# GuoleiSun/VSS-CFFM

Measured on AMD Instinct MI355X. Metric: clips/sec (fwd+bwd) CFFM-B1 480x480 T=4 hot path (CFFA+CFM, decoder_focal depth 2), higher is better.
Workload: dtype f32 in/out, f32 accumulate; MFMA operands: split-bf16 (hi+lo, ~2^-17) in the Linear GEMMs, f16 in QK^T/AV

## Files before the change

vss_cffm_amd/csrc/cffa_kernels.h:

```cpp
#pragma once
#include "cffm_common.h"

__device__ __forceinline__ void transpose_body(const float* __restrict__ src, float* __restrict__ dst,
                                               int rows, int cols, long src_bs, long dst_bs,
                                               const float* __restrict__ addend, int add_mod, int add_skip,
                                               float* __restrict__ copy_dst, int bx, int by, int bz) {
    __shared__ float tile[64][65];
    const int r0 = by * 64, c0 = bx * 64;
    const float* s = src + (long)bz * src_bs;
    float* d = dst + (long)bz * dst_bs;
    const int q = threadIdx.x & 15, p = threadIdx.x >> 4;
    const bool vin = (cols % 4 == 0) && (src_bs % 4 == 0) && (((uintptr_t)src & 15) == 0);
    const bool vout = (rows % 4 == 0) && (dst_bs % 4 == 0) && (((uintptr_t)dst & 15) == 0) && (((uintptr_t)addend & 15) == 0);
    const float* ad = (addend && (bz % add_mod) != add_skip) ? addend + (long)bz * dst_bs : nullptr;
    float* cp = (copy_dst && (bz % add_mod) != add_skip) ? copy_dst + (long)bz * src_bs : nullptr;
#pragma unroll
    for (int k = 0; k < 4; ++k) {
        const int r = r0 + p + 16 * k, c = c0 + 4 * q;
        f32x4 v = (f32x4){0.f, 0.f, 0.f, 0.f};
        if (r < rows) {
            if (vin && c + 3 < cols) {
                v = *(const f32x4*)(s + (long)r * cols + c);
                if (cp) *(f32x4*)(cp + (long)r * cols + c) = v;
            } else
                for (int e = 0; e < 4; ++e)
                    if (c + e < cols) { v[e] = s[(long)r * cols + c + e]; if (cp) cp[(long)r * cols + c + e] = v[e]; }
        }
#pragma unroll
        for (int e = 0; e < 4; ++e) tile[4 * q + e][p + 16 * k] = v[e];
    }
    __syncthreads();
#pragma unroll
    for (int k = 0; k < 4; ++k) {
        const int cl = p + 16 * k, c = c0 + cl, r = r0 + 4 * q;
        f32x4 v;
#pragma unroll
        for (int e = 0; e < 4; ++e) v[e] = tile[cl][4 * q + e];
        if (c < cols) {
            if (vout && r + 3 < rows) *(f32x4*)(d + (long)c * rows + r) = ad ? v + *(const f32x4*)(ad + (long)c * rows + r) : v;
            else
                for (int e = 0; e < 4; ++e)
                    if (r + e < rows) d[(long)c * rows + r + e] = v[e] + (ad ? ad[(long)c * rows + r + e] : 0.f);
        }
    }
}
__global__ void __launch_bounds__(256) k_transpose(const float* __restrict__ src, float* __restrict__ dst,
                                                    int rows, int cols, long src_bs, long dst_bs,
                                                    const float* __restrict__ addend, int add_mod, int add_skip,
                                                    float* __restrict__ copy_dst = nullptr) {
    transpose_body(src, dst, rows, cols, src_bs, dst_bs, addend, add_mod, add_skip, copy_dst, blockIdx.x, blockIdx.y, blockIdx.z);
}

__device__ __forceinline__ float bil_tap(int r, int p) {
    if (p == r) return (11.f - 2.f * r) * (1.f / 12.f);
    if (p == r + 1) return (1.f + 2.f * r) * (1.f / 12.f);
    return 0.f;
}

__device__ __forceinline__ void cell_geom(int g, int& grp, int& u, int& v, int& wsg) {
    if (g == 0) { grp = 0; u = v = 0; wsg = 7; }
    else if (g == 1) { grp = 1; u = v = 0; wsg = 7; }
    else if (g < 6) { grp = 2; u = (g - 2) >> 1; v = (g - 2) & 1; wsg = 3; }
    else { grp = 3; u = (g - 6) / 3; v = (g - 6) % 3; wsg = 2; }
}

struct PoolW { const float* w[4]; };
struct PoolWG { float* w[4]; float* b[4]; };

__device__ __forceinline__ float pool_matrix_entry(const PoolW& pw, int g, int i) {
    const int py = i / 7, px = i % 7;
    int grp, u, v, wsg;
    cell_geom(g, grp, u, v, wsg);
    if (grp < 2) return pw.w[grp][i];
    float m = 0.f;
    for (int a = 0; a < wsg; ++a)
        for (int b = 0; b < wsg; ++b)
            m += pw.w[grp][a * wsg + b] * bil_tap(wsg * u + a, py) * bil_tap(wsg * v + b, px);
    return m;
}
__device__ __forceinline__ void pool_matrix_body(const PoolW& pw, float* __restrict__ M) {
    for (int e = threadIdx.x; e < CFFM_NCELL * CFFM_WA; e += 256) M[e] = pool_matrix_entry(pw, e / CFFM_WA, e % CFFM_WA);
}

__global__ void __launch_bounds__(256) k_pool_matrix(PoolW pw, float* __restrict__ M) { pool_matrix_body(pw, M); }

__device__ __forceinline__ void pool_matrix_bwd_body(const float* __restrict__ dM, const PoolWG& gw, int t) {
    const int i = threadIdx.x;
    int grp, k;
    if (t < 49) { grp = 0; k = t; }
    else if (t < 98) { grp = 1; k = t - 49; }
    else if (t < 107) { grp = 2; k = t - 98; }
    else { grp = 3; k = t - 107; }
    float acc = 0.f;
    if (grp < 2) {
        if (i == k) acc = dM[grp * CFFM_WA + k];
    } else if (i < CFFM_WA) {
        const int wsg = grp == 2 ? 3 : 2, ncell = grp == 2 ? 2 : 3, g0 = grp == 2 ? 2 : 6;
        const int a = k / wsg, b = k % wsg;
        for (int u = 0; u < ncell; ++u)
            for (int v = 0; v < ncell; ++v)
                acc += dM[(g0 + u * ncell + v) * CFFM_WA + i] * bil_tap(wsg * u + a, i / 7) * bil_tap(wsg * v + b, i % 7);
    }
    acc = wave_sum(acc);
    if (i == 0) gw.w[grp][k] = acc;
    if (t == 0 && i < 3 && gw.b[0]) {
        gw.w[0][49 + i] = 0.f; gw.w[1][49 + i] = 0.f; gw.w[2][9 + i] = 0.f;
#pragma unroll
        for (int q = 0; q < 4; ++q) gw.b[q][1 + i] = 0.f;
    }
}
#define PMB_MAXD 4
struct PoolWGN { const float* dM[PMB_MAXD]; PoolWG gw[PMB_MAXD]; };
__global__ void __launch_bounds__(64) k_pool_matrix_bwd_n(PoolWGN a) { pool_matrix_bwd_body(a.dM[blockIdx.y], a.gw[blockIdx.y], blockIdx.x); }

struct Geo {
    int B, H0, W0, Hp, Wp, gy, gx, nW, HW, RC;
};
__device__ __forceinline__ int cell_row(const Geo& G, int wy, int wx, int g) {
    const int w = wy * G.gx + wx;
    if (g == 0) return 49 * G.nW + w;
    if (g == 1) return 50 * G.nW + w;
    if (g < 6) { int u = (g - 2) >> 1, v = (g - 2) & 1; return 51 * G.nW + (2 * wy + u) * (2 * G.gx) + 2 * wx + v; }
    int u = (g - 6) / 3, v = (g - 6) % 3;
    return 55 * G.nW + (3 * wy + u) * (3 * G.gx) + 3 * wx + v;
}
__device__ __forceinline__ void frame_cells(int frame, int& g0, int& ncell) {
    if (frame == 3) { g0 = 0; ncell = 1; }
    else if (frame == 0) { g0 = 1; ncell = 1; }
    else if (frame == 1) { g0 = 2; ncell = 4; }
    else { g0 = 6; ncell = 9; }
}

struct PoolB { const float* b[4]; };
struct PoolBG { float* b[4]; };
__device__ __forceinline__ int frame_group(int frame) { return frame == 3 ? 0 : frame + 1; }

#ifndef LNPF_BATCH
#define LNPF_BATCH 4
#endif
#ifndef LNP_WAVES
#define LNP_WAVES 8
#endif
#define LNP_THREADS (64 * LNP_WAVES)
#define LNP_PIX ((CFFM_WA + LNP_WAVES - 1) / LNP_WAVES)
template <bool INFER>
__global__ void __launch_bounds__(LNP_THREADS, 6) k_ln_pool_fwd(Geo G, const float* __restrict__ x_ref, long ref_bs,
                                                      const float* __restrict__ x_tgt, long tgt_bs,
                                                      const float* __restrict__ gamma, const float* __restrict__ beta,
                                                      const float* __restrict__ M , PoolW pw, PoolB pb,
                                                      float* __restrict__ zall, float* __restrict__ mean_out,
                                                      float* __restrict__ rstd_out, int split ) {
    __shared__ float sM[9 * CFFM_WA];
    __shared__ float red[4][9][CFFM_C];
    const int w = blockIdx.x, frame = blockIdx.y, b = blockIdx.z;
    const int wy = w / G.gx, wx = w % G.gx;
    const int lane = threadIdx.x & 63, wave = threadIdx.x >> 6;
    int g0, ncell;
    frame_cells(frame, g0, ncell);
    for (int e = threadIdx.x; e < ncell * CFFM_WA; e += LNP_THREADS)
        sM[e] = (INFER || M) ? M[g0 * CFFM_WA + e] : pool_matrix_entry(pw, g0 + e / CFFM_WA, e % CFFM_WA);
    __syncthreads();
    const float* xf = (frame == 3) ? x_tgt + (long)b * tgt_bs : x_ref + (long)b * ref_bs + (long)frame * G.HW * CFFM_C;
    const f32x4 gm = *(const f32x4*)(gamma + 4 * lane), bt = *(const f32x4*)(beta + 4 * lane);
    f32x4 acc[9];
#pragma unroll
    for (int c = 0; c < 9; ++c) acc[c] = (f32x4){0.f, 0.f, 0.f, 0.f};
#pragma unroll
    for (int k0 = 0; k0 < LNP_PIX; k0 += LNPF_BATCH) {
        f32x4 xr[LNPF_BATCH];
#pragma unroll
        for (int kk = 0; kk < LNPF_BATCH; ++kk) {
            const int i = wave + LNP_WAVES * (k0 + kk);
            const int y = 7 * wy + i / 7, x = 7 * wx + i % 7;
            xr[kk] = (f32x4){0.f, 0.f, 0.f, 0.f};
            if (k0 + kk < LNP_PIX && i < CFFM_WA && y < G.H0 && x < G.W0) xr[kk] = *(const f32x4*)(xf + ((long)y * G.W0 + x) * CFFM_C + 4 * lane);
        }
#pragma unroll
        for (int kk = 0; kk < LNPF_BATCH; ++kk) {
            const int i = wave + LNP_WAVES * (k0 + kk);
            if (k0 + kk >= LNP_PIX || i >= CFFM_WA) break;
            const int y = 7 * wy + i / 7, x = 7 * wx + i % 7;
            const bool valid = (y < G.H0) && (x < G.W0);
            f32x4 z = (f32x4){0.f, 0.f, 0.f, 0.f};
            if (valid) {
                const long pix = (long)y * G.W0 + x;
                const f32x4 xv = xr[kk];
                const float mu = wave_sum(xv[0] + xv[1] + xv[2] + xv[3]) * (1.f / CFFM_C);
                const f32x4 d = xv - mu;
                const float var = wave_sum(d[0] * d[0] + d[1] * d[1] + d[2] * d[2] + d[3] * d[3]) * (1.f / CFFM_C);
                const float rs = 1.f / sqrtf(var + CFFM_LN_EPS);
                z = d * rs * gm + bt;
                if (!INFER && lane == 0) {
                    mean_out[((long)b * 4 + frame) * G.HW + pix] = mu;
                    rstd_out[((long)b * 4 + frame) * G.HW + pix] = rs;
                }
            }
            if (frame == 3) *(f32x4*)(zall + ((long)b * G.RC + w * CFFM_WA + i) * CFFM_C + 4 * lane) = split ? split4_pack(z) : z;
            if (valid) {
#pragma unroll
                for (int c = 0; c < 9; ++c)
                    if (c < ncell) acc[c] += sM[c * CFFM_WA + i] * z;
            }
        }
    }
    static_assert(LNP_WAVES == 4 || LNP_WAVES == 8, "LNP_WAVES");
    if (wave < 4) {
#pragma unroll
        for (int c = 0; c < 9; ++c)
            if (c < ncell) *(f32x4*)(&red[wave][c][4 * lane]) = acc[c];
    }
    __syncthreads();
    if (LNP_WAVES == 8) {
        if (wave >= 4) {
#pragma unroll
            for (int c = 0; c < 9; ++c)
                if (c < ncell) *(f32x4*)(&red[wave - 4][c][4 * lane]) += acc[c];
        }
        __syncthreads();
    }
    const float pbias = pb.b[frame_group(frame)][0];
    if (!split) {
        for (int c = 0; c < ncell && threadIdx.x < CFFM_C; ++c) {
            const int ch = threadIdx.x;
            const float s = red[0][c][ch] + red[1][c][ch] + red[2][c][ch] + red[3][c][ch] + pbias;
            zall[((long)b * G.RC + cell_row(G, wy, wx, g0 + c)) * CFFM_C + ch] = s;
        }
    } else {
        for (int e = threadIdx.x; e < ncell * (CFFM_C / 4); e += LNP_THREADS) {
            const int c = e / (CFFM_C / 4), c4 = 4 * (e % (CFFM_C / 4));
            const f32x4 s = *(const f32x4*)(&red[0][c][c4]) + *(const f32x4*)(&red[1][c][c4]) + *(const f32x4*)(&red[2][c][c4]) +
                            *(const f32x4*)(&red[3][c][c4]) + pbias;
            *(f32x4*)(zall + ((long)b * G.RC + cell_row(G, wy, wx, g0 + c)) * CFFM_C + c4) = split4_pack(s);
        }
    }
}

#define LNP_RSTRIDE 1216
#define LNP_TAIL_TGT (CFFM_WA + 1)
#define LNP_TAIL_REF (14 * CFFM_WA + 3)
#ifndef LNB_SPLIT
#define LNB_SPLIT 4
#endif
#ifndef LNB_WAVES
#define LNB_WAVES 4
#endif
#define LNB_THREADS (64 * LNB_WAVES)
#define LNB_PIX ((CFFM_WA + LNB_SPLIT * LNB_WAVES - 1) / (LNB_SPLIT * LNB_WAVES))

__device__ __forceinline__ float dot4(f32x4 a, f32x4 b) { return a[0] * b[0] + a[1] * b[1] + a[2] * b[2] + a[3] * b[3]; }

__global__ void __launch_bounds__(LNB_THREADS) k_ln_pool_bwd_tgt(Geo G, const float* __restrict__ x_tgt, long tgt_bs,
                                                                 const float* __restrict__ gamma, const float* __restrict__ beta,
                                                                 const float* __restrict__ M, const float* __restrict__ mean_in,
                                                                 const float* __restrict__ rstd_in, const float* __restrict__ dzall,
                                                                 const float* __restrict__ dres, float* __restrict__ dx_tgt, long dtgt_bs,
                                                                 float* __restrict__ rec) {
    __shared__ float red[LNB_WAVES][2][CFFM_C];
    __shared__ float sdM[CFFM_WA];
    __shared__ float sbs;
    const int s = blockIdx.x % LNB_SPLIT, wb = blockIdx.x / LNB_SPLIT;
    const int w = wb % G.nW, b = wb / G.nW;
    const int wy = w / G.gx, wx = w % G.gx;
    const int lane = threadIdx.x & 63, wave = wave_uniform(threadIdx.x >> 6);
    const float* xf = x_tgt + (long)b * tgt_bs;
    float* dxf = dx_tgt + (long)b * dtgt_bs;
    if (threadIdx.x < CFFM_WA) sdM[threadIdx.x] = 0.f;
    f32x4 xr[LNB_PIX], dzr[LNB_PIX], addr[LNB_PIX];
    float mur[LNB_PIX], rsr[LNB_PIX], m0[LNB_PIX];
#pragma unroll
    for (int k = 0; k < LNB_PIX; ++k) {
        const int i = s + LNB_SPLIT * (wave + LNB_WAVES * k);
        const int y = 7 * wy + i / 7, x = 7 * wx + i % 7;
        xr[k] = dzr[k] = addr[k] = (f32x4){0.f, 0.f, 0.f, 0.f};
        mur[k] = rsr[k] = m0[k] = 0.f;
        if (i < CFFM_WA && y < G.H0 && x < G.W0) {
            const long pix = (long)y * G.W0 + x;
            xr[k] = *(const f32x4*)(xf + pix * CFFM_C + 4 * lane);
            mur[k] = mean_in[((long)b * 4 + 3) * G.HW + pix];
            rsr[k] = rstd_in[((long)b * 4 + 3) * G.HW + pix];
            m0[k] = M[i];
            dzr[k] = *(const f32x4*)(dzall + ((long)b * G.RC + w * CFFM_WA + i) * CFFM_C + 4 * lane);
            if (dres) addr[k] = *(const f32x4*)(dres + ((long)b * G.HW + pix) * CFFM_C + 4 * lane);
        }
    }
    const f32x4 dp = *(const f32x4*)(dzall + ((long)b * G.RC + cell_row(G, wy, wx, 0)) * CFFM_C + 4 * lane);
    const f32x4 gm = *(const f32x4*)(gamma + 4 * lane), bt = *(const f32x4*)(beta + 4 * lane);
    if (wave == 0) {
        const float bs = wave_sum(dp[0] + dp[1] + dp[2] + dp[3]);
        if (lane == 0) sbs = (s == 0) ? bs : 0.f;
    }
    f32x4 ag = (f32x4){0.f, 0.f, 0.f, 0.f}, ab = (f32x4){0.f, 0.f, 0.f, 0.f};
    __syncthreads();
#pragma unroll
    for (int k = 0; k < LNB_PIX; ++k) {
        const int i = s + LNB_SPLIT * (wave + LNB_WAVES * k);
        if (i >= CFFM_WA) break;
        const int y = 7 * wy + i / 7, x = 7 * wx + i % 7;
        if (!((y < G.H0) && (x < G.W0))) continue;
        const long pix = (long)y * G.W0 + x;
        const float rs = rsr[k];
        const f32x4 xh = (xr[k] - mur[k]) * rs;
        const f32x4 z = xh * gm + bt;
        const f32x4 dz = dzr[k] + m0[k] * dp;
        const float dm = wave_sum_hi(dot4(dp, z));
        if (lane == 63) sdM[i] = dm;
        ag += dz * xh;
        ab += dz;
        const f32x4 gz = dz * gm;
        const float m1 = wave_sum(gz[0] + gz[1] + gz[2] + gz[3]) * (1.f / CFFM_C);
        const float m2 = wave_sum(dot4(gz, xh)) * (1.f / CFFM_C);
        const f32x4 dx = (gz - m1 - xh * m2) * rs + addr[k];
        *(f32x4*)(dxf + pix * CFFM_C + 4 * lane) = dx;
    }
    *(f32x4*)(&red[wave][0][4 * lane]) = ag;
    *(f32x4*)(&red[wave][1][4 * lane]) = ab;
    __syncthreads();
    float* r = rec + (long)blockIdx.x * LNP_RSTRIDE;
    for (int e = threadIdx.x; e < 2 * CFFM_C; e += LNB_THREADS) {
        const int which = e / CFFM_C, ch = e % CFFM_C;
        float t = red[0][which][ch];
#pragma unroll
        for (int q = 1; q < LNB_WAVES; ++q) t += red[q][which][ch];
        r[e] = t;
    }
    if (threadIdx.x < CFFM_WA) r[2 * CFFM_C + threadIdx.x] = sdM[threadIdx.x];
    if (threadIdx.x == CFFM_WA) r[2 * CFFM_C + CFFM_WA] = sbs;
}

#define RB_MAXD 4
struct CffaRefBlocks {
    int n;
    const float* gamma[RB_MAXD];
    const float* beta[RB_MAXD];
    const float* M[RB_MAXD];
    const float* dzall[RB_MAXD];
    float* rec[RB_MAXD];
};
#define RB_LDS_BLOCK (14 * CFFM_C + 2 * 14 * CFFM_WA)
__host__ __device__ constexpr int cffa_ref_lds(int D) {
    return 4 * ((D * RB_LDS_BLOCK > LNB_WAVES * D * 2 * CFFM_C + 14 * D * CFFM_WA ? D * RB_LDS_BLOCK : LNB_WAVES * D * 2 * CFFM_C + 14 * D * CFFM_WA) + 4 * D + 4);
}

struct RefRows { f32x4 x[LNB_PIX], add[LNB_PIX]; float mu[LNB_PIX], rs[LNB_PIX]; };
template <bool ACC>
__device__ __forceinline__ void ln_pool_ref_load(RefRows& R, const Geo& G, const float* __restrict__ xf, const float* __restrict__ dxf,
                                                 const float* __restrict__ mean_f, const float* __restrict__ rstd_f, int s, int wy, int wx,
                                                 int lane, int wave) {
#pragma unroll
    for (int k = 0; k < LNB_PIX; ++k) {
        const int i = s + LNB_SPLIT * (wave + LNB_WAVES * k);
        const int y = 7 * wy + i / 7, x = 7 * wx + i % 7;
        R.x[k] = R.add[k] = (f32x4){0.f, 0.f, 0.f, 0.f};
        R.mu[k] = R.rs[k] = 0.f;
        if (i < CFFM_WA && y < G.H0 && x < G.W0) {
            const long pix = (long)y * G.W0 + x;
            R.x[k] = *(const f32x4*)(xf + pix * CFFM_C + 4 * lane);
            R.mu[k] = mean_f[pix];
            R.rs[k] = rstd_f[pix];
            if (ACC) R.add[k] = *(const f32x4*)(dxf + pix * CFFM_C + 4 * lane);
        }
    }
}
template <int NC, int D>
__device__ __forceinline__ void ln_pool_bwd_ref_frame(const Geo& G, const RefRows& R, float* __restrict__ dxf,
                                                      const float* sP, const float* sMm, float* sdM, const f32x4 (&gm)[D], const f32x4 (&bt)[D],
                                                      f32x4 (&ag)[D], f32x4 (&ab)[D], int g0, int s, int wy, int wx, int lane, int wave) {
#pragma unroll
    for (int k = 0; k < LNB_PIX; ++k) {
        const int i = s + LNB_SPLIT * (wave + LNB_WAVES * k);
        if (i >= CFFM_WA) break;
        const int y = 7 * wy + i / 7, x = 7 * wx + i % 7;
        if (!((y < G.H0) && (x < G.W0))) continue;
        const long pix = (long)y * G.W0 + x;
        const float rs = R.rs[k];
        const f32x4 xh = (R.x[k] - R.mu[k]) * rs;
        f32x4 gz = (f32x4){0.f, 0.f, 0.f, 0.f};
        constexpr int NCD = NC == 9 ? 3 : (NC == 4 ? 2 : 1), WSG = NC == 9 ? 2 : (NC == 4 ? 3 : 7);
        const int iy = i / 7, ix = i % 7;
        int u0 = 0, u1 = 0, v0 = 0, v1 = 0;
        if (NC > 1) {
            u0 = (iy > 0 ? iy - 1 : 0) / WSG; u1 = (iy < 5 ? iy : 5) / WSG;
            v0 = (ix > 0 ? ix - 1 : 0) / WSG; v1 = (ix < 5 ? ix : 5) / WSG;
        }
#pragma unroll
        for (int d = 0; d < D; ++d) {
            const f32x4 z = xh * gm[d] + bt[d];
            f32x4 dz = (f32x4){0.f, 0.f, 0.f, 0.f};
            for (int u = u0; u <= u1; ++u)
                for (int v = v0; v <= v1; ++v) {
                    const int c = d * 14 + g0 - 1 + u * NCD + v;
                    const f32x4 dp = *(const f32x4*)(sP + c * CFFM_C + 4 * lane);
                    dz += sMm[c * CFFM_WA + i] * dp;
                    const float dm = wave_sum_hi(dot4(dp, z));
                    if (lane == 63) sdM[c * CFFM_WA + i] = dm;
                }
            ag[d] += dz * xh;
            ab[d] += dz;
            gz += dz * gm[d];
        }
        const float m1 = wave_sum(gz[0] + gz[1] + gz[2] + gz[3]) * (1.f / CFFM_C);
        const float m2 = wave_sum(dot4(gz, xh)) * (1.f / CFFM_C);
        const f32x4 dx = (gz - m1 - xh * m2) * rs + R.add[k];
        *(f32x4*)(dxf + pix * CFFM_C + 4 * lane) = dx;
    }
}

template <int D, bool ACC>
__global__ void __launch_bounds__(LNB_THREADS) k_ln_pool_bwd_ref(Geo G, const float* __restrict__ x_ref, long ref_bs, CffaRefBlocks Bk,
                                                                 const float* __restrict__ mean_in, const float* __restrict__ rstd_in,
                                                                 float* __restrict__ dx_ref, long dref_bs) {
    CFFM_DYN_SMEM(smem);
    float* sP = (float*)smem;
    float* sMm = sP + D * 14 * CFFM_C;
    float* red = (float*)smem;
    constexpr int body = D * (14 * CFFM_C + 14 * CFFM_WA), redn = LNB_WAVES * D * 2 * CFFM_C;
    float* sdM = (float*)smem + (body > redn ? body : redn);
    float* sbs = sdM + D * 14 * CFFM_WA;
    const int s = blockIdx.x % LNB_SPLIT, wb = blockIdx.x / LNB_SPLIT;
    const int w = wb % G.nW, b = wb / G.nW;
    const int wy = w / G.gx, wx = w % G.gx;
    const int lane = threadIdx.x & 63, wave = wave_uniform(threadIdx.x >> 6);
    for (int e = threadIdx.x; e < D * 14 * CFFM_WA; e += LNB_THREADS) {
        const int d = e / (14 * CFFM_WA), r = e % (14 * CFFM_WA);
        sMm[e] = Bk.M[d][CFFM_WA + r];
        sdM[e] = 0.f;
    }
    for (int r = wave; r < D * 14; r += LNB_WAVES) {
        const int d = r / 14, c = r % 14;
        *(f32x4*)(sP + r * CFFM_C + 4 * lane) = *(const f32x4*)(Bk.dzall[d] + ((long)b * G.RC + cell_row(G, wy, wx, 1 + c)) * CFFM_C + 4 * lane);
    }
    f32x4 gm[D], bt[D], ag[D], ab[D];
#pragma unroll
    for (int d = 0; d < D; ++d) {
        gm[d] = *(const f32x4*)(Bk.gamma[d] + 4 * lane);
        bt[d] = *(const f32x4*)(Bk.beta[d] + 4 * lane);
        ag[d] = ab[d] = (f32x4){0.f, 0.f, 0.f, 0.f};
    }
    __syncthreads();
    if (s == 0) {
        for (int q = wave; q < 3 * D; q += LNB_WAVES) {
            const int d = q / 3, grp = q % 3;
            const int c0 = grp == 0 ? 0 : (grp == 1 ? 1 : 5), nc = grp == 0 ? 1 : (grp == 1 ? 4 : 9);
            float t = 0.f;
            for (int c = 0; c < nc; ++c) {
                const f32x4 v = *(const f32x4*)(sP + (d * 14 + c0 + c) * CFFM_C + 4 * lane);
                t += v[0] + v[1] + v[2] + v[3];
            }
            t = wave_sum(t);
            if (lane == 0) sbs[d * 4 + grp] = t;
        }
    } else if (threadIdx.x < 4 * D) sbs[threadIdx.x] = 0.f;
    const float* xb = x_ref + (long)b * ref_bs;
    float* dxb = dx_ref + (long)b * dref_bs;
    const long fr = (long)G.HW * CFFM_C;
    const float* mb = mean_in + (long)b * 4 * G.HW;
    const float* rb = rstd_in + (long)b * 4 * G.HW;
    RefRows Ra, Rb;
    ln_pool_ref_load<ACC>(Ra, G, xb, dxb, mb, rb, s, wy, wx, lane, wave);
    ln_pool_ref_load<ACC>(Rb, G, xb + fr, dxb + fr, mb + G.HW, rb + G.HW, s, wy, wx, lane, wave);
    ln_pool_bwd_ref_frame<1, D>(G, Ra, dxb, sP, sMm, sdM, gm, bt, ag, ab, 1, s, wy, wx, lane, wave);
    ln_pool_ref_load<ACC>(Ra, G, xb + 2 * fr, dxb + 2 * fr, mb + 2 * G.HW, rb + 2 * G.HW, s, wy, wx, lane, wave);
    ln_pool_bwd_ref_frame<4, D>(G, Rb, dxb + fr, sP, sMm, sdM, gm, bt, ag, ab, 2, s, wy, wx, lane, wave);
    ln_pool_bwd_ref_frame<9, D>(G, Ra, dxb + 2 * fr, sP, sMm, sdM, gm, bt, ag, ab, 6, s, wy, wx, lane, wave);
    __syncthreads();
#pragma unroll
    for (int d = 0; d < D; ++d) {
        *(f32x4*)(red + ((wave * D + d) * 2 + 0) * CFFM_C + 4 * lane) = ag[d];
        *(f32x4*)(red + ((wave * D + d) * 2 + 1) * CFFM_C + 4 * lane) = ab[d];
    }
    __syncthreads();
    for (int d = 0; d < D; ++d) {
        float* r = Bk.rec[d] + (long)blockIdx.x * LNP_RSTRIDE;
        for (int e = threadIdx.x; e < 2 * CFFM_C; e += LNB_THREADS) {
            float t = red[(d * 2) * CFFM_C + e];
#pragma unroll
            for (int q = 1; q < LNB_WAVES; ++q) t += red[((q * D + d) * 2) * CFFM_C + e];
            r[e] = t;
        }
        for (int e = threadIdx.x; e < LNP_TAIL_REF; e += LNB_THREADS)
            r[2 * CFFM_C + e] = e < 14 * CFFM_WA ? sdM[d * 14 * CFFM_WA + e] : sbs[d * 4 + (e - 14 * CFFM_WA)];
    }
}
```

Before: 2914.

## Process one pixel per 16-lane quad in LN-pool backward kernels

Restructures the LN-pool backward kernels so that each 16-lane group of a wave owns one pixel, with every lane holding four f32x4 channel chunks. Reductions become row16 sums instead of full-wave reductions, and per-pixel loops turn into parallel lanes. The ref kernel also stages gamma/beta in LDS, unrolls over fixed candidate cells with pinned accumulators, and computes the beta-gradient algebraically from summed pooling weights rather than accumulating dz per pixel. In exchange it adds barrier-serialised quad reductions into LDS and more registers per lane, now capped by a launch-bounds occupancy hint.

Result: no change. 2897 (median of 2 runs) (-0.6%).

```diff
diff --git a/vss_cffm_amd/csrc/cffa_kernels.h b/vss_cffm_amd/csrc/cffa_kernels.h
--- a/vss_cffm_amd/csrc/cffa_kernels.h
+++ b/vss_cffm_amd/csrc/cffa_kernels.h
@@ -246,8 +246,24 @@
 #endif
 #define LNB_THREADS (64 * LNB_WAVES)
 #define LNB_PIX ((CFFM_WA + LNB_SPLIT * LNB_WAVES - 1) / (LNB_SPLIT * LNB_WAVES))
+static_assert(LNB_PIX <= 4, "a wave's pixels must fit one quad (four 16-lane groups)");
 
 __device__ __forceinline__ float dot4(f32x4 a, f32x4 b) { return a[0] * b[0] + a[1] * b[1] + a[2] * b[2] + a[3] * b[3]; }
+__device__ __forceinline__ float sum4(f32x4 a) { return a[0] + a[1] + a[2] + a[3]; }
+
+__device__ __forceinline__ void quad_reduce_to_lds(float* dst, const f32x4 (&v)[4], int q, int j) {
+#pragma unroll
+    for (int p = 0; p < 4; ++p) {
+        if (q == p) {
+#pragma unroll
+            for (int t = 0; t < 4; ++t) {
+                f32x4* a = (f32x4*)(dst + 4 * j + 64 * t);
+                *a = p == 0 ? v[t] : *a + v[t];
+            }
+        }
+        __syncthreads();
+    }
+}
 
 __global__ void __launch_bounds__(LNB_THREADS) k_ln_pool_bwd_tgt(Geo G, const float* __restrict__ x_tgt, long tgt_bs,
                                                                  const float* __restrict__ gamma, const float* __restrict__ beta,
@@ -262,65 +278,70 @@
     const int w = wb % G.nW, b = wb / G.nW;
     const int wy = w / G.gx, wx = w % G.gx;
     const int lane = threadIdx.x & 63, wave = wave_uniform(threadIdx.x >> 6);
+    const int q = lane >> 4, j = lane & 15;
     const float* xf = x_tgt + (long)b * tgt_bs;
     float* dxf = dx_tgt + (long)b * dtgt_bs;
     if (threadIdx.x < CFFM_WA) sdM[threadIdx.x] = 0.f;
-    f32x4 xr[LNB_PIX], dzr[LNB_PIX], addr[LNB_PIX];
-    float mur[LNB_PIX], rsr[LNB_PIX], m0[LNB_PIX];
-#pragma unroll
-    for (int k = 0; k < LNB_PIX; ++k) {
-        const int i = s + LNB_SPLIT * (wave + LNB_WAVES * k);
-        const int y = 7 * wy + i / 7, x = 7 * wx + i % 7;
-        xr[k] = dzr[k] = addr[k] = (f32x4){0.f, 0.f, 0.f, 0.f};
-        mur[k] = rsr[k] = m0[k] = 0.f;
-        if (i < CFFM_WA && y < G.H0 && x < G.W0) {
-            const long pix = (long)y * G.W0 + x;
-            xr[k] = *(const f32x4*)(xf + pix * CFFM_C + 4 * lane);
-            mur[k] = mean_in[((long)b * 4 + 3) * G.HW + pix];
-            rsr[k] = rstd_in[((long)b * 4 + 3) * G.HW + pix];
-            m0[k] = M[i];
-            dzr[k] = *(const f32x4*)(dzall + ((long)b * G.RC + w * CFFM_WA + i) * CFFM_C + 4 * lane);
-            if (dres) addr[k] = *(const f32x4*)(dres + ((long)b * G.HW + pix) * CFFM_C + 4 * lane);
-        }
-    }
-    const f32x4 dp = *(const f32x4*)(dzall + ((long)b * G.RC + cell_row(G, wy, wx, 0)) * CFFM_C + 4 * lane);
-    const f32x4 gm = *(const f32x4*)(gamma + 4 * lane), bt = *(const f32x4*)(beta + 4 * lane);
+    const int i = s + LNB_SPLIT * (wave + LNB_WAVES * q);
+    const int y = 7 * wy + i / 7, x = 7 * wx + i % 7;
+    const bool valid = q < LNB_PIX && i < CFFM_WA && y < G.H0 && x < G.W0;
+    const long pix = (long)y * G.W0 + x;
+    f32x4 xr[4], dzr[4], addr[4], dp[4], gm[4], bt[4];
+    float mu = 0.f, rs = 0.f, m0 = 0.f;
+#pragma unroll
+    for (int t = 0; t < 4; ++t) {
+        const int c = 4 * j + 64 * t;
+        xr[t] = dzr[t] = addr[t] = (f32x4){0.f, 0.f, 0.f, 0.f};
+        if (valid) {
+            xr[t] = *(const f32x4*)(xf + pix * CFFM_C + c);
+            dzr[t] = *(const f32x4*)(dzall + ((long)b * G.RC + w * CFFM_WA + i) * CFFM_C + c);
+            if (dres) addr[t] = *(const f32x4*)(dres + ((long)b * G.HW + pix) * CFFM_C + c);
+        }
+        dp[t] = *(const f32x4*)(dzall + ((long)b * G.RC + cell_row(G, wy, wx, 0)) * CFFM_C + c);
+        gm[t] = *(const f32x4*)(gamma + c);
+        bt[t] = *(const f32x4*)(beta + c);
+    }
+    if (valid) {
+        mu = mean_in[((long)b * 4 + 3) * G.HW + pix];
+        rs = rstd_in[((long)b * 4 + 3) * G.HW + pix];
+        m0 = M[i];
+    }
     if (wave == 0) {
-        const float bs = wave_sum(dp[0] + dp[1] + dp[2] + dp[3]);
+        const float bs = row16_sum(sum4(dp[0]) + sum4(dp[1]) + sum4(dp[2]) + sum4(dp[3]));
         if (lane == 0) sbs = (s == 0) ? bs : 0.f;
     }
-    f32x4 ag = (f32x4){0.f, 0.f, 0.f, 0.f}, ab = (f32x4){0.f, 0.f, 0.f, 0.f};
-    __syncthreads();
-#pragma unroll
-    for (int k = 0; k < LNB_PIX; ++k) {
-        const int i = s + LNB_SPLIT * (wave + LNB_WAVES * k);
-        if (i >= CFFM_WA) break;
-        const int y = 7 * wy + i / 7, x = 7 * wx + i % 7;
-        if (!((y < G.H0) && (x < G.W0))) continue;
-        const long pix = (long)y * G.W0 + x;
-        const float rs = rsr[k];
-        const f32x4 xh = (xr[k] - mur[k]) * rs;
-        const f32x4 z = xh * gm + bt;
-        const f32x4 dz = dzr[k] + m0[k] * dp;
-        const float dm = wave_sum_hi(dot4(dp, z));
-        if (lane == 63) sdM[i] = dm;
-        ag += dz * xh;
-        ab += dz;
-        const f32x4 gz = dz * gm;
-        const float m1 = wave_sum(gz[0] + gz[1] + gz[2] + gz[3]) * (1.f / CFFM_C);
-        const float m2 = wave_sum(dot4(gz, xh)) * (1.f / CFFM_C);
-        const f32x4 dx = (gz - m1 - xh * m2) * rs + addr[k];
-        *(f32x4*)(dxf + pix * CFFM_C + 4 * lane) = dx;
-    }
-    *(f32x4*)(&red[wave][0][4 * lane]) = ag;
-    *(f32x4*)(&red[wave][1][4 * lane]) = ab;
-    __syncthreads();
+    __syncthreads();
+    f32x4 ag[4], ab[4], xh[4], gz[4];
+    float pdm = 0.f, p1 = 0.f, p2 = 0.f;
+#pragma unroll
+    for (int t = 0; t < 4; ++t) {
+        xh[t] = (xr[t] - mu) * rs;
+        const f32x4 z = xh[t] * gm[t] + bt[t];
+        const f32x4 dz = dzr[t] + m0 * dp[t];
+        pdm += dot4(dp[t], z);
+        ag[t] = dz * xh[t];
+        ab[t] = dz;
+        gz[t] = dz * gm[t];
+        p1 += sum4(gz[t]);
+        p2 += dot4(gz[t], xh[t]);
+    }
+    const float dm = row16_sum(pdm);
+    const float m1 = row16_sum(p1) * (1.f / CFFM_C);
+    const float m2 = row16_sum(p2) * (1.f / CFFM_C);
+    if (valid) {
+        if (j == 0) sdM[i] = dm;
+#pragma unroll
+        for (int t = 0; t < 4; ++t)
+            *(f32x4*)(dxf + pix * CFFM_C + 4 * j + 64 * t) = (gz[t] - m1 - xh[t] * m2) * rs + addr[t];
+    }
+    quad_reduce_to_lds(&red[wave][0][0], ag, q, j);
+    quad_reduce_to_lds(&red[wave][1][0], ab, q, j);
     float* r = rec + (long)blockIdx.x * LNP_RSTRIDE;
     for (int e = threadIdx.x; e < 2 * CFFM_C; e += LNB_THREADS) {
         const int which = e / CFFM_C, ch = e % CFFM_C;
         float t = red[0][which][ch];
 #pragma unroll
-        for (int q = 1; q < LNB_WAVES; ++q) t += red[q][which][ch];
+        for (int k = 1; k < LNB_WAVES; ++k) t += red[k][which][ch];
         r[e] = t;
     }
     if (threadIdx.x < CFFM_WA) r[2 * CFFM_C + threadIdx.x] = sdM[threadIdx.x];
@@ -336,110 +357,167 @@
     const float* dzall[RB_MAXD];
     float* rec[RB_MAXD];
 };
-#define RB_LDS_BLOCK (14 * CFFM_C + 2 * 14 * CFFM_WA)
+#define RB_LDS_BLOCK (14 * CFFM_C + 2 * 14 * CFFM_WA + 2 * CFFM_C)
 __host__ __device__ constexpr int cffa_ref_lds(int D) {
-    return 4 * ((D * RB_LDS_BLOCK > LNB_WAVES * D * 2 * CFFM_C + 14 * D * CFFM_WA ? D * RB_LDS_BLOCK : LNB_WAVES * D * 2 * CFFM_C + 14 * D * CFFM_WA) + 4 * D + 4);
-}
-
-struct RefRows { f32x4 x[LNB_PIX], add[LNB_PIX]; float mu[LNB_PIX], rs[LNB_PIX]; };
+    return 4 * (D * RB_LDS_BLOCK + 4 * D + 14 * D + 4);
+}
+
+#ifdef CFFM_EMU
+#define LNB_PIN(v)
+#else
+#define LNB_PIN(v) asm volatile("" : "+v"(v))
+#endif
+struct RefRows { f32x4 x[4], add[4]; float mu, rs; };
 template <bool ACC>
-__device__ __forceinline__ void ln_pool_ref_load(RefRows& R, const Geo& G, const float* __restrict__ xf, const float* __restrict__ dxf,
-                                                 const float* __restrict__ mean_f, const float* __restrict__ rstd_f, int s, int wy, int wx,
-                                                 int lane, int wave) {
-#pragma unroll
-    for (int k = 0; k < LNB_PIX; ++k) {
-        const int i = s + LNB_SPLIT * (wave + LNB_WAVES * k);
-        const int y = 7 * wy + i / 7, x = 7 * wx + i % 7;
-        R.x[k] = R.add[k] = (f32x4){0.f, 0.f, 0.f, 0.f};
-        R.mu[k] = R.rs[k] = 0.f;
-        if (i < CFFM_WA && y < G.H0 && x < G.W0) {
-            const long pix = (long)y * G.W0 + x;
-            R.x[k] = *(const f32x4*)(xf + pix * CFFM_C + 4 * lane);
-            R.mu[k] = mean_f[pix];
-            R.rs[k] = rstd_f[pix];
-            if (ACC) R.add[k] = *(const f32x4*)(dxf + pix * CFFM_C + 4 * lane);
-        }
+__device__ __forceinline__ void ln_pool_ref_load(RefRows& R, const float* __restrict__ xf, const float* __restrict__ dxf,
+                                                 const float* __restrict__ mean_f, const float* __restrict__ rstd_f, bool valid, long pix, int j) {
+    R.mu = R.rs = 0.f;
+#pragma unroll
+    for (int t = 0; t < 4; ++t) {
+        R.x[t] = R.add[t] = (f32x4){0.f, 0.f, 0.f, 0.f};
+        if (valid) {
+            R.x[t] = *(const f32x4*)(xf + pix * CFFM_C + 4 * j + 64 * t);
+            if (ACC) R.add[t] = *(const f32x4*)(dxf + pix * CFFM_C + 4 * j + 64 * t);
+        }
+    }
+    if (valid) {
+        R.mu = mean_f[pix];
+        R.rs = rstd_f[pix];
     }
 }
 template <int NC, int D>
-__device__ __forceinline__ void ln_pool_bwd_ref_frame(const Geo& G, const RefRows& R, float* __restrict__ dxf,
-                                                      const float* sP, const float* sMm, float* sdM, const f32x4 (&gm)[D], const f32x4 (&bt)[D],
-                                                      f32x4 (&ag)[D], f32x4 (&ab)[D], int g0, int s, int wy, int wx, int lane, int wave) {
-#pragma unroll
-    for (int k = 0; k < LNB_PIX; ++k) {
-        const int i = s + LNB_SPLIT * (wave + LNB_WAVES * k);
-        if (i >= CFFM_WA) break;
-        const int y = 7 * wy + i / 7, x = 7 * wx + i % 7;
-        if (!((y < G.H0) && (x < G.W0))) continue;
-        const long pix = (long)y * G.W0 + x;
-        const float rs = R.rs[k];
-        const f32x4 xh = (R.x[k] - R.mu[k]) * rs;
-        f32x4 gz = (f32x4){0.f, 0.f, 0.f, 0.f};
-        constexpr int NCD = NC == 9 ? 3 : (NC == 4 ? 2 : 1), WSG = NC == 9 ? 2 : (NC == 4 ? 3 : 7);
-        const int iy = i / 7, ix = i % 7;
-        int u0 = 0, u1 = 0, v0 = 0, v1 = 0;
-        if (NC > 1) {
-            u0 = (iy > 0 ? iy - 1 : 0) / WSG; u1 = (iy < 5 ? iy : 5) / WSG;
-            v0 = (ix > 0 ? ix - 1 : 0) / WSG; v1 = (ix < 5 ? ix : 5) / WSG;
-        }
+__device__ __forceinline__ void ln_pool_bwd_ref_frame(const RefRows& R, float* __restrict__ dxf, const float* sP, const float* sMm,
+                                                      const float* sGB, float* sdM, f32x4 (&ag)[D][4], int g0, int i,
+                                                      bool valid, long pix, int j) {
+    constexpr int NCD = NC == 9 ? 3 : (NC == 4 ? 2 : 1), WSG = NC == 9 ? 2 : (NC == 4 ? 3 : 7), NCAND = NC == 1 ? 1 : 4;
+    const int ii = valid ? i : 0, iy = ii / 7, ix = ii % 7;
+    int u0 = 0, u1 = 0, v0 = 0, v1 = 0;
+    if (NC > 1) {
+        u0 = (iy > 0 ? iy - 1 : 0) / WSG; u1 = (iy < 5 ? iy : 5) / WSG;
+        v0 = (ix > 0 ? ix - 1 : 0) / WSG; v1 = (ix < 5 ? ix : 5) / WSG;
+    }
+    int cc[NCAND];
+    bool sees[NCAND];
+#pragma unroll
+    for (int n = 0; n < NCAND; ++n) {
+        int u = 0, v = 0;
+        if (NC == 4) { u = n >> 1; v = n & 1; sees[n] = valid && u >= u0 && u <= u1 && v >= v0 && v <= v1; }
+        else if (NC == 9) { u = u0 + (n >> 1); v = v0 + (n & 1); sees[n] = valid && u <= u1 && v <= v1; }
+        else sees[n] = valid;
+        cc[n] = sees[n] ? g0 - 1 + u * NCD + v : g0 - 1;
+    }
+    float wt[D][NCAND], pdm[D][NCAND];
+#pragma unroll
+    for (int d = 0; d < D; ++d)
+#pragma unroll
+        for (int n = 0; n < NCAND; ++n) {
+            wt[d][n] = sees[n] ? sMm[(d * 14 + cc[n]) * CFFM_WA + ii] : 0.f;
+            pdm[d][n] = 0.f;
+        }
+    const float rs = R.rs;
+    f32x4 xh[4], gz[4];
+    float p1 = 0.f, p2 = 0.f;
+#pragma unroll
+    for (int t = 0; t < 4; ++t) {
+        const int ch = 4 * j + 64 * t;
+        xh[t] = (R.x[t] - R.mu) * rs;
+        gz[t] = (f32x4){0.f, 0.f, 0.f, 0.f};
 #pragma unroll
         for (int d = 0; d < D; ++d) {
-            const f32x4 z = xh * gm[d] + bt[d];
+            const f32x4 gm = *(const f32x4*)(sGB + (2 * d) * CFFM_C + ch), bt = *(const f32x4*)(sGB + (2 * d + 1) * CFFM_C + ch);
+            const f32x4 z = xh[t] * gm + bt;
             f32x4 dz = (f32x4){0.f, 0.f, 0.f, 0.f};
-            for (int u = u0; u <= u1; ++u)
-                for (int v = v0; v <= v1; ++v) {
-                    const int c = d * 14 + g0 - 1 + u * NCD + v;
-                    const f32x4 dp = *(const f32x4*)(sP + c * CFFM_C + 4 * lane);
-                    dz += sMm[c * CFFM_WA + i] * dp;
-                    const float dm = wave_sum_hi(dot4(dp, z));
-                    if (lane == 63) sdM[c * CFFM_WA + i] = dm;
-                }
-            ag[d] += dz * xh;
-            ab[d] += dz;
-            gz += dz * gm[d];
-        }
-        const float m1 = wave_sum(gz[0] + gz[1] + gz[2] + gz[3]) * (1.f / CFFM_C);
-        const float m2 = wave_sum(dot4(gz, xh)) * (1.f / CFFM_C);
-        const f32x4 dx = (gz - m1 - xh * m2) * rs + R.add[k];
-        *(f32x4*)(dxf + pix * CFFM_C + 4 * lane) = dx;
+#pragma unroll
+            for (int n = 0; n < NCAND; ++n) {
+                const f32x4 dp = *(const f32x4*)(sP + (d * 14 + cc[n]) * CFFM_C + ch);
+                dz += wt[d][n] * dp;
+                pdm[d][n] += dot4(dp, z);
+                LNB_PIN(pdm[d][n]);
+            }
+            ag[d][t] += dz * xh[t];
+            LNB_PIN(ag[d][t]);
+            gz[t] += dz * gm;
+        }
+        LNB_PIN(gz[t]);
+        p1 += sum4(gz[t]);
+        p2 += dot4(gz[t], xh[t]);
+        LNB_PIN(p1);
+        LNB_PIN(p2);
+    }
+#pragma unroll
+    for (int d = 0; d < D; ++d)
+#pragma unroll
+        for (int n = 0; n < NCAND; ++n) {
+            const float dm = row16_sum(pdm[d][n]);
+            if (sees[n] && j == 0) sdM[(d * 14 + cc[n]) * CFFM_WA + ii] = dm;
+        }
+    const float m1 = row16_sum(p1) * (1.f / CFFM_C);
+    const float m2 = row16_sum(p2) * (1.f / CFFM_C);
+    if (valid) {
+#pragma unroll
+        for (int t = 0; t < 4; ++t)
+            *(f32x4*)(dxf + pix * CFFM_C + 4 * j + 64 * t) = (gz[t] - m1 - xh[t] * m2) * rs + R.add[t];
     }
 }
 
 template <int D, bool ACC>
-__global__ void __launch_bounds__(LNB_THREADS) k_ln_pool_bwd_ref(Geo G, const float* __restrict__ x_ref, long ref_bs, CffaRefBlocks Bk,
+__global__ void __launch_bounds__(LNB_THREADS, (D <= 2 ? 3 : (D == 3 ? 2 : 1))) k_ln_pool_bwd_ref(Geo G, const float* __restrict__ x_ref, long ref_bs, CffaRefBlocks Bk,
                                                                  const float* __restrict__ mean_in, const float* __restrict__ rstd_in,
                                                                  float* __restrict__ dx_ref, long dref_bs) {
     CFFM_DYN_SMEM(smem);
     float* sP = (float*)smem;
-    float* sMm = sP + D * 14 * CFFM_C;
+    float* sGB = sP + D * 14 * CFFM_C;
+    float* sMm = sGB + D * 2 * CFFM_C;
     float* red = (float*)smem;
-    constexpr int body = D * (14 * CFFM_C + 14 * CFFM_WA), redn = LNB_WAVES * D * 2 * CFFM_C;
+    constexpr int body = D * (14 * CFFM_C + 14 * CFFM_WA + 2 * CFFM_C), redn = LNB_WAVES * D * CFFM_C;
     float* sdM = (float*)smem + (body > redn ? body : redn);
     float* sbs = sdM + D * 14 * CFFM_WA;
+    float* scw = sbs + 4 * D;
     const int s = blockIdx.x % LNB_SPLIT, wb = blockIdx.x / LNB_SPLIT;
     const int w = wb % G.nW, b = wb / G.nW;
     const int wy = w / G.gx, wx = w % G.gx;
     const int lane = threadIdx.x & 63, wave = wave_uniform(threadIdx.x >> 6);
+    const int q = lane >> 4, j = lane & 15;
     for (int e = threadIdx.x; e < D * 14 * CFFM_WA; e += LNB_THREADS) {
         const int d = e / (14 * CFFM_WA), r = e % (14 * CFFM_WA);
         sMm[e] = Bk.M[d][CFFM_WA + r];
         sdM[e] = 0.f;
     }
+    for (int e = threadIdx.x; e < D * 2 * CFFM_C; e += LNB_THREADS) {
+        const int d = e / (2 * CFFM_C), r = e % (2 * CFFM_C);
+        sGB[e] = r < CFFM_C ? Bk.gamma[d][r] : Bk.beta[d][r - CFFM_C];
+    }
     for (int r = wave; r < D * 14; r += LNB_WAVES) {
         const int d = r / 14, c = r % 14;
         *(f32x4*)(sP + r * CFFM_C + 4 * lane) = *(const f32x4*)(Bk.dzall[d] + ((long)b * G.RC + cell_row(G, wy, wx, 1 + c)) * CFFM_C + 4 * lane);
     }
-    f32x4 gm[D], bt[D], ag[D], ab[D];
-#pragma unroll
-    for (int d = 0; d < D; ++d) {
-        gm[d] = *(const f32x4*)(Bk.gamma[d] + 4 * lane);
-        bt[d] = *(const f32x4*)(Bk.beta[d] + 4 * lane);
-        ag[d] = ab[d] = (f32x4){0.f, 0.f, 0.f, 0.f};
-    }
-    __syncthreads();
+    const int i = s + LNB_SPLIT * (wave + LNB_WAVES * q);
+    const int y = 7 * wy + i / 7, x = 7 * wx + i % 7;
+    const bool valid = q < LNB_PIX && i < CFFM_WA && y < G.H0 && x < G.W0;
+    const long pix = (long)y * G.W0 + x;
+    const float* xb = x_ref + (long)b * ref_bs;
+    float* dxb = dx_ref + (long)b * dref_bs;
+    const long fr = (long)G.HW * CFFM_C;
+    const float* mb = mean_in + (long)b * 4 * G.HW;
+    const float* rb = rstd_in + (long)b * 4 * G.HW;
+    RefRows Ra, Rb;
+    ln_pool_ref_load<ACC>(Ra, xb, dxb, mb, rb, valid, pix, j);
+    ln_pool_ref_load<ACC>(Rb, xb + fr, dxb + fr, mb + G.HW, rb + G.HW, valid, pix, j);
+    f32x4 ag[D][4];
+#pragma unroll
+    for (int d = 0; d < D; ++d)
+#pragma unroll
+        for (int t = 0; t < 4; ++t) ag[d][t] = (f32x4){0.f, 0.f, 0.f, 0.f};
+    __syncthreads();
+    for (int e = threadIdx.x; e < D * 14; e += LNB_THREADS) {
+        float t = 0.f;
+        for (int k = s; k < CFFM_WA; k += LNB_SPLIT)
+            if (7 * wy + k / 7 < G.H0 && 7 * wx + k % 7 < G.W0) t += sMm[e * CFFM_WA + k];
+        scw[e] = t;
+    }
     if (s == 0) {
-        for (int q = wave; q < 3 * D; q += LNB_WAVES) {
-            const int d = q / 3, grp = q % 3;
+        for (int k = wave; k < 3 * D; k += LNB_WAVES) {
+            const int d = k / 3, grp = k % 3;
             const int c0 = grp == 0 ? 0 : (grp == 1 ? 1 : 5), nc = grp == 0 ? 1 : (grp == 1 ? 4 : 9);
             float t = 0.f;
             for (int c = 0; c < nc; ++c) {
@@ -450,31 +528,27 @@
             if (lane == 0) sbs[d * 4 + grp] = t;
         }
     } else if (threadIdx.x < 4 * D) sbs[threadIdx.x] = 0.f;
-    const float* xb = x_ref + (long)b * ref_bs;
-    float* dxb = dx_ref + (long)b * dref_bs;
-    const long fr = (long)G.HW * CFFM_C;
-    const float* mb = mean_in + (long)b * 4 * G.HW;
-    const float* rb = rstd_in + (long)b * 4 * G.HW;
-    RefRows Ra, Rb;
-    ln_pool_ref_load<ACC>(Ra, G, xb, dxb, mb, rb, s, wy, wx, lane, wave);
-    ln_pool_ref_load<ACC>(Rb, G, xb + fr, dxb + fr, mb + G.HW, rb + G.HW, s, wy, wx, lane, wave);
-    ln_pool_bwd_ref_frame<1, D>(G, Ra, dxb, sP, sMm, sdM, gm, bt, ag, ab, 1, s, wy, wx, lane, wave);
-    ln_pool_ref_load<ACC>(Ra, G, xb + 2 * fr, dxb + 2 * fr, mb + 2 * G.HW, rb + 2 * G.HW, s, wy, wx, lane, wave);
-    ln_pool_bwd_ref_frame<4, D>(G, Rb, dxb + fr, sP, sMm, sdM, gm, bt, ag, ab, 2, s, wy, wx, lane, wave);
-    ln_pool_bwd_ref_frame<9, D>(G, Ra, dxb + 2 * fr, sP, sMm, sdM, gm, bt, ag, ab, 6, s, wy, wx, lane, wave);
-    __syncthreads();
-#pragma unroll
-    for (int d = 0; d < D; ++d) {
-        *(f32x4*)(red + ((wave * D + d) * 2 + 0) * CFFM_C + 4 * lane) = ag[d];
-        *(f32x4*)(red + ((wave * D + d) * 2 + 1) * CFFM_C + 4 * lane) = ab[d];
-    }
-    __syncthreads();
+    ln_pool_bwd_ref_frame<1, D>(Ra, dxb, sP, sMm, sGB, sdM, ag, 1, i, valid, pix, j);
+    ln_pool_ref_load<ACC>(Ra, xb + 2 * fr, dxb + 2 * fr, mb + 2 * G.HW, rb + 2 * G.HW, valid, pix, j);
+    ln_pool_bwd_ref_frame<4, D>(Rb, dxb + fr, sP, sMm, sGB, sdM, ag, 2, i, valid, pix, j);
+    ln_pool_bwd_ref_frame<9, D>(Ra, dxb + 2 * fr, sP, sMm, sGB, sdM, ag, 6, i, valid, pix, j);
+    __syncthreads();
+    for (int e = threadIdx.x; e < D * CFFM_C; e += LNB_THREADS) {
+        const int d = e / CFFM_C, ch = e % CFFM_C;
+        float t = 0.f;
+#pragma unroll
+        for (int c = 0; c < 14; ++c) t += scw[d * 14 + c] * sP[(d * 14 + c) * CFFM_C + ch];
+        Bk.rec[d][(long)blockIdx.x * LNP_RSTRIDE + CFFM_C + ch] = t;
+    }
+    __syncthreads();
+#pragma unroll
+    for (int d = 0; d < D; ++d) quad_reduce_to_lds(red + (wave * D + d) * CFFM_C, ag[d], q, j);
     for (int d = 0; d < D; ++d) {
         float* r = Bk.rec[d] + (long)blockIdx.x * LNP_RSTRIDE;
-        for (int e = threadIdx.x; e < 2 * CFFM_C; e += LNB_THREADS) {
-            float t = red[(d * 2) * CFFM_C + e];
-#pragma unroll
-            for (int q = 1; q < LNB_WAVES; ++q) t += red[((q * D + d) * 2) * CFFM_C + e];
+        for (int e = threadIdx.x; e < CFFM_C; e += LNB_THREADS) {
+            float t = red[d * CFFM_C + e];
+#pragma unroll
+            for (int k = 1; k < LNB_WAVES; ++k) t += red[(k * D + d) * CFFM_C + e];
             r[e] = t;
         }
         for (int e = threadIdx.x; e < LNP_TAIL_REF; e += LNB_THREADS)
```
